# jmoraispk/DeepMIMO

Measured on AMD Instinct MI355X. Metric: user-channels/sec, higher is better.
Workload: dtype f16x3-split MFMA, f32 accumulate

## Files before the change

deepmimo_amd/csrc/k2_channel_fd_fold.hip:

```cpp
#include "dmx_common.h"
#include "dmx_tuning.h"

namespace dmx {

typedef _Float16 fh8 __attribute__((ext_vector_type(8)));
typedef _Float16 fh2 __attribute__((ext_vector_type(2)));
typedef __fp16 fhp2 __attribute__((ext_vector_type(2)));
typedef float ff16 __attribute__((ext_vector_type(16)));
typedef unsigned fu4 __attribute__((ext_vector_type(4)));

static constexpr int FOLD_TROW = 272;
static constexpr float FOLD_B_SCALE = 64.0f;
static constexpr int FOLD_MAX_M = 128;
static constexpr int FOLD_SHARED_FROM = 33;
static constexpr size_t FOLD_MIN_LDS = 160 * 1024 / 5 + 64;

struct FoldArgs {
    int64_t user_begin;
    int m_tx, ue_mh, bs_mh;
    int M, K;
    int sc_first, sc_stride;
    double inv_n;
    int ch;
    int sch;
    int nblk;
    int nchunk;
    int nsuper;
    int nb_last;
    int tab_rows;
    int adaptive;
    int k_tail;
    int mlog;
};

typedef float fv2 __attribute__((ext_vector_type(2)));

__device__ __forceinline__ void fold_split2(float x0, float x1, fh2& hi, fh2& lo, float m1) {
    const fhp2 h = __builtin_amdgcn_cvt_pkrtz(x0, x1);
    const fh2 hh = __builtin_bit_cast(fh2, h);
    const float r0 = __builtin_fmaf((float)hh[0], m1, x0);
    const float r1 = __builtin_fmaf((float)hh[1], m1, x1);
    const fhp2 l = __builtin_amdgcn_cvt_pkrtz(r0, r1);
    hi = hh;
    lo = __builtin_bit_cast(fh2, l);
}

__device__ __forceinline__ unsigned fold_bits(float x) { return __builtin_bit_cast(unsigned, x); }

__device__ __forceinline__ float fold_max_paths(float v) {
    int x = __builtin_bit_cast(int, v);
    v = fmaxf(v, __builtin_bit_cast(float, __builtin_amdgcn_update_dpp(x, x, 0xB1, 0xF, 0xF, false)));
    x = __builtin_bit_cast(int, v);
    v = fmaxf(v, __builtin_bit_cast(float, __builtin_amdgcn_update_dpp(x, x, 0x4E, 0xF, 0xF, false)));
    x = __builtin_bit_cast(int, v);
    v = fmaxf(v, __builtin_bit_cast(float, __builtin_amdgcn_update_dpp(x, x, 0x141, 0xF, 0xF, false)));
    x = __builtin_bit_cast(int, v);
    v = fmaxf(v, __builtin_bit_cast(float, __builtin_amdgcn_update_dpp(x, x, 0x140, 0xF, 0xF, false)));
    x = __builtin_bit_cast(int, v);
    return fmaxf(__builtin_bit_cast(float, __builtin_amdgcn_readlane(x, 0)), __builtin_bit_cast(float, __builtin_amdgcn_readlane(x, 16)));
}

__device__ __forceinline__ void wave_lds_sync() {
    __builtin_amdgcn_fence(__ATOMIC_ACQ_REL, "workgroup");
    __builtin_amdgcn_wave_barrier();
}

__host__ __device__ inline size_t fold_static_bytes(int tab_rows, int M) { return (size_t)tab_rows * 12 + align_up((size_t)M * 4, 16); }
__host__ __device__ inline size_t fold_wave_bytes(int M, int ch) { return 256 + (size_t)(M + ch) * FOLD_TROW; }

template <int WS>
__device__ __forceinline__ void fold_sync() {
    if constexpr (WS == 4) __syncthreads();
    else wave_lds_sync();
}


typedef float ff4 __attribute__((ext_vector_type(4)));
struct FoldX { ff4 x0, x1, y0, y1; };
#define FOLD_X_IO(X) "+{v[112:115]}"((X).x0), "+{v[116:119]}"((X).x1), "+{v[120:123]}"((X).y0), "+{v[124:127]}"((X).y1)

__device__ __forceinline__ uint32_t fold_lds_addr(const void* p) {
    return (uint32_t)(size_t)(__attribute__((address_space(3))) const void*)p;
}

__device__ __forceinline__ void fold_load0(FoldX& X, uint32_t ar, uint32_t er) {
    asm volatile(
        "ds_read_b128 v[112:115], %4\n\t"
        "ds_read_b128 v[116:119], %4 offset:16\n\t"
        "ds_read_b128 v[120:123], %5\n\t"
        "ds_read_b128 v[124:127], %5 offset:16"
        : "={v[112:115]}"(X.x0), "={v[116:119]}"(X.x1), "={v[120:123]}"(X.y0), "={v[124:127]}"(X.y1)
        : "v"(ar), "v"(er));
}

__device__ __forceinline__ void fold_drain(FoldX& X) { asm volatile("s_waitcnt lgkmcnt(0)" : FOLD_X_IO(X)); }

#define FOLD_CMUL_TEXT                                                                                               \
    "s_waitcnt lgkmcnt(0)\n\t"                                                                                       \
    "v_pk_mul_f32 v[108:109], v[112:113], v[120:121] op_sel:[1,1] op_sel_hi:[1,0]\n\t"                                \
    "v_pk_mul_f32 v[110:111], v[114:115], v[122:123] op_sel:[1,1] op_sel_hi:[1,0]\n\t"                                \
    "v_pk_fma_f32 v[112:113], v[112:113], v[120:121], v[108:109] op_sel_hi:[0,1,1] neg_lo:[0,0,1]\n\t"                \
    "v_pk_fma_f32 v[114:115], v[114:115], v[122:123], v[110:111] op_sel_hi:[0,1,1] neg_lo:[0,0,1]\n\t"                \
    "v_pk_mul_f32 v[108:109], v[116:117], v[124:125] op_sel:[1,1] op_sel_hi:[1,0]\n\t"                                \
    "v_pk_mul_f32 v[110:111], v[118:119], v[126:127] op_sel:[1,1] op_sel_hi:[1,0]\n\t"                                \
    "v_pk_fma_f32 v[116:117], v[116:117], v[124:125], v[108:109] op_sel_hi:[0,1,1] neg_lo:[0,0,1]\n\t"                \
    "v_pk_fma_f32 v[118:119], v[118:119], v[126:127], v[110:111] op_sel_hi:[0,1,1] neg_lo:[0,0,1]\n\t"
#define FOLD_CVT_HI_TEXT                                                                                             \
    "v_cvt_pkrtz_f16_f32 %0, v112, v113\n\t"                                                                         \
    "v_cvt_pkrtz_f16_f32 %1, v114, v115\n\t"                                                                         \
    "v_cvt_pkrtz_f16_f32 %2, v116, v117\n\t"                                                                         \
    "v_cvt_pkrtz_f16_f32 %3, v118, v119\n\t"
template <bool LO, int OFF>
__device__ __forceinline__ void fold_kstep(FoldX& X, float m1, uint32_t ar, uint32_t er, fh8& Ah, fh8& Al) {
    unsigned h0, h1, h2, h3;
    if constexpr (LO) {
        unsigned l0, l1, l2, l3;
        asm volatile(
            FOLD_CMUL_TEXT
            FOLD_CVT_HI_TEXT
            "v_fma_mix_f32 v112, %0, %14, v112 op_sel_hi:[1,0,0]\n\t"
            "v_fma_mix_f32 v113, %0, %14, v113 op_sel:[1,0,0] op_sel_hi:[1,0,0]\n\t"
            "v_fma_mix_f32 v114, %1, %14, v114 op_sel_hi:[1,0,0]\n\t"
            "v_fma_mix_f32 v115, %1, %14, v115 op_sel:[1,0,0] op_sel_hi:[1,0,0]\n\t"
            "v_fma_mix_f32 v116, %2, %14, v116 op_sel_hi:[1,0,0]\n\t"
            "v_fma_mix_f32 v117, %2, %14, v117 op_sel:[1,0,0] op_sel_hi:[1,0,0]\n\t"
            "v_fma_mix_f32 v118, %3, %14, v118 op_sel_hi:[1,0,0]\n\t"
            "v_fma_mix_f32 v119, %3, %14, v119 op_sel:[1,0,0] op_sel_hi:[1,0,0]\n\t"
            "v_cvt_pkrtz_f16_f32 %4, v112, v113\n\t"
            "v_cvt_pkrtz_f16_f32 %5, v114, v115\n\t"
            "v_cvt_pkrtz_f16_f32 %6, v116, v117\n\t"
            "v_cvt_pkrtz_f16_f32 %7, v118, v119\n\t"
            "ds_read_b128 v[112:115], %12 offset:%15\n\t"
            "ds_read_b128 v[116:119], %12 offset:%16\n\t"
            "ds_read_b128 v[120:123], %13 offset:%15\n\t"
            "ds_read_b128 v[124:127], %13 offset:%16"
            : "=&v"(h0), "=&v"(h1), "=&v"(h2), "=&v"(h3), "=&v"(l0), "=&v"(l1), "=&v"(l2), "=&v"(l3), FOLD_X_IO(X)
            : "v"(ar), "v"(er), "s"(m1), "i"(OFF), "i"(OFF + 16)
            : "v108", "v109", "v110", "v111");
        Al = __builtin_bit_cast(fh8, fu4{l0, l1, l2, l3});
    } else {
        asm volatile(
            FOLD_CMUL_TEXT
            FOLD_CVT_HI_TEXT
            "ds_read_b128 v[112:115], %8 offset:%10\n\t"
            "ds_read_b128 v[116:119], %8 offset:%11\n\t"
            "ds_read_b128 v[120:123], %9 offset:%10\n\t"
            "ds_read_b128 v[124:127], %9 offset:%11"
            : "=&v"(h0), "=&v"(h1), "=&v"(h2), "=&v"(h3), FOLD_X_IO(X)
            : "v"(ar), "v"(er), "i"(OFF), "i"(OFF + 16)
            : "v108", "v109", "v110", "v111");
    }
    Ah = __builtin_bit_cast(fh8, fu4{h0, h1, h2, h3});
    if constexpr (!LO) Al = Ah;
}
#undef FOLD_CMUL_TEXT
#undef FOLD_CVT_HI_TEXT

__device__ __forceinline__ uint32_t fold_rowbits_off(uint32_t r, int mlog, uint32_t K8) {
    return (r & ((1u << mlog) - 1u)) * K8 + ((r >> mlog) << 7);
}

template <int NS>
__device__ __forceinline__ void fold_finish(ff16& acc0, ff16& acc1, fv2 osc, fv2 (&w)[8]) {
    if constexpr (NS > 1) {
        asm volatile("s_nop 15" : "+v"(acc0), "+v"(acc1));
        fv2 t[8];
#pragma unroll
        for (int i = 0; i < 8; ++i) {
            const fv2 a = {acc0[2 * i], acc0[2 * i + 1]}, b = {acc1[2 * i], acc1[2 * i + 1]};
            asm volatile("v_pk_add_f32 %0, %1, %2" : "=v"(t[i]) : "v"(a), "v"(b));
        }
#pragma unroll
        for (int i = 0; i < 8; ++i) asm volatile("v_pk_mul_f32 %0, %1, %2" : "=v"(w[i]) : "v"(t[i]), "v"(osc));
    } else {
        asm volatile("s_nop 15" : "+v"(acc0));
#pragma unroll
        for (int i = 0; i < 8; ++i) {
            const fv2 a = {acc0[2 * i], acc0[2 * i + 1]};
            asm volatile("v_pk_mul_f32 %0, %1, %2" : "=v"(w[i]) : "v"(a), "v"(osc));
        }
    }
}

template <int S, int NS, bool LW>
__device__ __forceinline__ void fold_ksteps(FoldX& X, float m1, uint32_t ar, uint32_t er, uint32_t arn, uint32_t ern,
                                            ff16& acc0, ff16& acc1, const fh8 (&Bhi)[4], const fh8 (&Blo)[4]) {
    constexpr bool weak = LW && S == NS - 1;
    fh8 Ah, Al;
    if constexpr (S == NS - 1) fold_kstep<!weak, 0>(X, m1, arn, ern, Ah, Al);
    else fold_kstep<true, (S + 1) * 64>(X, m1, ar, er, Ah, Al);
    __builtin_amdgcn_sched_barrier(0);
    if constexpr (S & 1) {
        acc1 = __builtin_amdgcn_mfma_f32_32x32x16_f16(Ah, Bhi[S], acc1, 0, 0, 0);
        if constexpr (!weak) {
            acc1 = __builtin_amdgcn_mfma_f32_32x32x16_f16(Ah, Blo[S], acc1, 0, 0, 0);
            acc1 = __builtin_amdgcn_mfma_f32_32x32x16_f16(Al, Bhi[S], acc1, 0, 0, 0);
        }
    } else {
        acc0 = __builtin_amdgcn_mfma_f32_32x32x16_f16(Ah, Bhi[S], acc0, 0, 0, 0);
        if constexpr (!weak) {
            acc0 = __builtin_amdgcn_mfma_f32_32x32x16_f16(Ah, Blo[S], acc0, 0, 0, 0);
            acc0 = __builtin_amdgcn_mfma_f32_32x32x16_f16(Al, Bhi[S], acc0, 0, 0, 0);
        }
    }
    __builtin_amdgcn_sched_barrier(0);
    if constexpr (S + 1 < NS) fold_ksteps<S + 1, NS, LW>(X, m1, ar, er, arn, ern, acc0, acc1, Bhi, Blo);
}

struct FoldStoreCtx {
    __amdgpu_buffer_rsrc_t orsrc;
    uint32_t lane_col;
    uint32_t lane_row;
    uint32_t lmask_last;
    uint32_t K8;
    int mlog;
    int nb;
    int lane_hh;
    int tail_lane_dead;
    bool masked;
};

template <bool NT, int WS, int NS, bool LW, bool SROW>
__device__ __forceinline__ void fold_tiles(int sub, int ntiles, const uint32_t* rowsrc, const uint32_t* rowoff, int lp, int hh,
                                           const unsigned char* Ac, const unsigned char* E1, const fh8 (&Bhi)[4], const fh8 (&Blo)[4],
                                           float m1, fv2 osc, const FoldStoreCtx& c) {
    if (sub >= ntiles) return;
    constexpr int AUX = NT ? 2 : 0;
    const int rows = c.nb << (SROW ? c.mlog : 0);
    const int rt_chk = !SROW ? 0 : (c.masked ? (((c.nb - 1) << c.mlog) >> 5) : ((rows & 31) ? ntiles - 1 : ntiles));
    uint32_t P[4], D[4];
    if constexpr (SROW) {
#pragma unroll
        for (int q = 0; q < 4; ++q) { P[q] = fold_rowbits_off((uint32_t)q, c.mlog, c.K8); D[q] = fold_rowbits_off((uint32_t)(8 * q), c.mlog, c.K8); }
    }
    const uint32_t ac_lds = fold_lds_addr(Ac) + (uint32_t)hh * 32u, e1_lds = fold_lds_addr(E1) + (uint32_t)hh * 32u;
    uint32_t src = rowsrc[(sub << 5) + lp];
    uint32_t ar = ac_lds + (src >> 16), er = e1_lds + (src & 0xFFFFu);
    FoldX X;
    fold_load0(X, ar, er);
    for (int rt = sub; rt < ntiles; rt += WS) {
        const int rtn = rt + WS < ntiles ? rt + WS : rt;
        const uint32_t srcn = rowsrc[(rtn << 5) + lp];
        const uint32_t arn = ac_lds + (srcn >> 16), ern = e1_lds + (srcn & 0xFFFFu);
        ff16 acc0, acc1;
#pragma unroll
        for (int i = 0; i < 16; ++i) { acc0[i] = 0.f; acc1[i] = 0.f; }
        fold_ksteps<0, NS, LW>(X, m1, ar, er, arn, ern, acc0, acc1, Bhi, Blo);
        ar = arn; er = ern;
        fv2 w[8];
        fold_finish<NS>(acc0, acc1, osc, w);
        if constexpr (SROW) {
            const uint32_t T = fold_rowbits_off((uint32_t)rt << 5, c.mlog, c.K8);
            if (rt < rt_chk) {
#pragma unroll
                for (int i = 0; i < 16; ++i)
                    __builtin_amdgcn_raw_buffer_store_b32(fold_bits(w[i >> 1][i & 1]), c.orsrc, c.lane_row, T + P[i & 3] + D[i >> 2], AUX);
            } else {
#pragma unroll
                for (int i = 0; i < 16; ++i) {
                    const int a_blk = ((rt << 5) + (i & 3) + 8 * (i >> 2) + 4 * c.lane_hh) >> c.mlog;
                    const bool dead = a_blk >= c.nb || (c.masked && a_blk == c.nb - 1 && c.tail_lane_dead);
                    __builtin_amdgcn_raw_buffer_store_b32(fold_bits(w[i >> 1][i & 1]), c.orsrc, dead ? 0x80000000u : c.lane_row,
                                                          T + P[i & 3] + D[i >> 2], AUX);
                }
            }
        } else {
            const uint4* ro4 = reinterpret_cast<const uint4*>(rowoff + (rt << 5) + 4 * hh);
            if (c.masked) {
#pragma unroll
                for (int g = 0; g < 4; ++g) {
                    const uint4 ro = ro4[2 * g];
                    __builtin_amdgcn_raw_buffer_store_b32(fold_bits(w[2 * g][0]), c.orsrc, c.lane_col + (ro.x & c.lmask_last), 0, AUX);
                    __builtin_amdgcn_raw_buffer_store_b32(fold_bits(w[2 * g][1]), c.orsrc, c.lane_col + (ro.y & c.lmask_last), 0, AUX);
                    __builtin_amdgcn_raw_buffer_store_b32(fold_bits(w[2 * g + 1][0]), c.orsrc, c.lane_col + (ro.z & c.lmask_last), 0, AUX);
                    __builtin_amdgcn_raw_buffer_store_b32(fold_bits(w[2 * g + 1][1]), c.orsrc, c.lane_col + (ro.w & c.lmask_last), 0, AUX);
                }
            } else {
#pragma unroll
                for (int g = 0; g < 4; ++g) {
                    const uint4 ro = ro4[2 * g];
                    __builtin_amdgcn_raw_buffer_store_b32(fold_bits(w[2 * g][0]), c.orsrc, c.lane_col + ro.x, 0, AUX);
                    __builtin_amdgcn_raw_buffer_store_b32(fold_bits(w[2 * g][1]), c.orsrc, c.lane_col + ro.y, 0, AUX);
                    __builtin_amdgcn_raw_buffer_store_b32(fold_bits(w[2 * g + 1][0]), c.orsrc, c.lane_col + ro.z, 0, AUX);
                    __builtin_amdgcn_raw_buffer_store_b32(fold_bits(w[2 * g + 1][1]), c.orsrc, c.lane_col + ro.w, 0, AUX);
                }
            }
        }
    }
    fold_drain(X);
}

template <bool NT, int WS, bool SROW>
__device__ __forceinline__ void fold_tiles_kind(int tile_kind, int sub, int ntiles, const uint32_t* rowsrc, const uint32_t* rowoff, int lp, int hh,
                                                const unsigned char* Ac, const unsigned char* E1, const fh8 (&Bhi)[4], const fh8 (&Blo)[4],
                                                float m1, fv2 osc, const FoldStoreCtx& c) {
    switch (tile_kind) {
        case 2: fold_tiles<NT, WS, 1, false, SROW>(sub, ntiles, rowsrc, rowoff, lp, hh, Ac, E1, Bhi, Blo, m1, osc, c); break;
        case 4: fold_tiles<NT, WS, 2, false, SROW>(sub, ntiles, rowsrc, rowoff, lp, hh, Ac, E1, Bhi, Blo, m1, osc, c); break;
        case 5: fold_tiles<NT, WS, 2, true, SROW>(sub, ntiles, rowsrc, rowoff, lp, hh, Ac, E1, Bhi, Blo, m1, osc, c); break;
        case 6: fold_tiles<NT, WS, 3, false, SROW>(sub, ntiles, rowsrc, rowoff, lp, hh, Ac, E1, Bhi, Blo, m1, osc, c); break;
        case 7: fold_tiles<NT, WS, 3, true, SROW>(sub, ntiles, rowsrc, rowoff, lp, hh, Ac, E1, Bhi, Blo, m1, osc, c); break;
        case 8: fold_tiles<NT, WS, 4, false, SROW>(sub, ntiles, rowsrc, rowoff, lp, hh, Ac, E1, Bhi, Blo, m1, osc, c); break;
        default: fold_tiles<NT, WS, 4, true, SROW>(sub, ntiles, rowsrc, rowoff, lp, hh, Ac, E1, Bhi, Blo, m1, osc, c); break;
    }
}

template <bool NT, int WS>
__global__ __launch_bounds__(256, 4) void k2_fd_fold(WsView ws, FoldArgs a, float* __restrict__ out, int64_t items) {
    extern __shared__ __attribute__((aligned(16))) unsigned char smem[];
    uint32_t* rowoff0 = reinterpret_cast<uint32_t*>(smem);
    uint32_t* rowoff1 = rowoff0 + a.tab_rows;
    uint32_t* rowsrc = rowoff1 + a.tab_rows;
    uint32_t* pidx = rowsrc + a.tab_rows;
    const int tid = threadIdx.x, lane = tid & 63;
    const int wave = __builtin_amdgcn_readfirstlane(tid >> 6);
    unsigned char* wbase = smem + fold_static_bytes(a.tab_rows, a.M) + (WS == 1 ? (size_t)wave * fold_wave_bytes(a.M, a.ch) : (size_t)0);
    float2* qtab = reinterpret_cast<float2*>(wbase);
    unsigned char* Ac = wbase + 256;
    unsigned char* E1 = Ac + (size_t)a.M * FOLD_TROW;

    const int M = a.M, K = a.K;
    for (int r = tid; r < a.tab_rows; r += 256) {
        const int ab = r / M, p = r - ab * M;
        const uint32_t off = (uint32_t)(p * K + 16 * ab) * 8u;
        const int nb0 = a.nchunk > 1 ? a.ch : a.nb_last;
        rowoff0[r] = ab < nb0 ? off : 0xC0000000u;
        uint32_t o1 = ab < a.nb_last ? off : 0xC0000000u;
        if (ab == a.nb_last - 1 && a.k_tail < 16) o1 |= 0x80000000u;
        rowoff1[r] = o1;
        const bool any = ab < (a.ch > a.nb_last ? a.ch : a.nb_last);
        rowsrc[r] = any ? ((uint32_t)(ab * FOLD_TROW) | ((uint32_t)(p * FOLD_TROW) << 16)) : 0u;
    }
    for (int p = tid; p < M; p += 256) {
        const int rx = p / a.m_tx, tx = p - rx * a.m_tx;
        pidx[p] = (uint32_t)(rx % a.ue_mh) | ((uint32_t)(rx / a.ue_mh) << 8) | ((uint32_t)(tx % a.bs_mh) << 16) |
                  ((uint32_t)(tx / a.bs_mh) << 24);
    }
    __syncthreads();

    const int lp = lane & 31, hh = lane >> 5;
    const int col = lane & 31, bsc = col >> 1, cpart = col & 1;
    const int kb = a.sc_stride * bsc;
    const float kbl = (float)(kb & 4095), kbf = (float)kb, cq = 0.25f * (float)cpart;
    const uint32_t lane_col = (uint32_t)col * 4u;
    const uint32_t lmask_last = bsc < a.k_tail ? 0x7FFFFFFFu : 0xFFFFFFFFu;
    const size_t user_floats = (size_t)M * K * 2;

    constexpr int IW = 4 / WS;
    const int sub = WS == 4 ? wave : 0;
    for (int64_t item = (int64_t)blockIdx.x * IW + (WS == 1 ? wave : 0); item < items; item += (int64_t)gridDim.x * IW) {
        const int64_t ul = a.nsuper == 1 ? item : item / a.nsuper;
        const int sc = a.nsuper == 1 ? 0 : (int)(item - ul * a.nsuper);
        const int64_t u = a.user_begin + ul;
        const int b0 = sc * a.sch;
        const int bn = (a.nblk - b0) < a.sch ? (a.nblk - b0) : a.sch;
        int n_act = ws.n_keep[u];
        n_act = n_act < 32 ? n_act : 32;
        if (n_act == 0) {
            float* __restrict__ oz = out + (size_t)ul * user_floats + (size_t)b0 * 32;
            const int k0 = b0 * 16, k1 = (k0 + bn * 16) < K ? (k0 + bn * 16) : K;
            const int nfl = (k1 - k0) * 2;
            for (int p = sub; p < M; p += WS)
                for (int i = lane; i < nfl; i += 64) oz[(size_t)p * K * 2 + i] = 0.f;
            continue;
        }
        const size_t rb = (size_t)u * ws.P + lp;
        const bool ok = lp < n_act;
        const float cr = ok ? ws.c_re[rb] : 0.f, ci = ok ? ws.c_im[rb] : 0.f;
        const double q = ok ? (double)ws.dn[rb] * a.inv_n : 0.0;
        const double rxy = ok ? ws.rx_y[rb] : 0.0, rxz = ok ? ws.rx_z[rb] : 0.0;
        const double txy = ok ? ws.tx_y[rb] : 0.0, txz = ok ? ws.tx_z[rb] : 0.0;
        const float m = fold_max_paths(fmaxf(fabsf(cr), fabsf(ci)));
        bool last_weak = false;
        if (a.adaptive) {
            const int l0w = ((n_act - 1) >> 3) << 3;
            const float a2 = fmaf(cr, cr, ci * ci);
            const float m2 = fold_max_paths(a2), mw2 = fold_max_paths(lp >= l0w ? a2 : 0.f);
            last_weak = l0w >= 8 && mw2 * 4194304.0f <= m2;
        }
        int e;
        (void)frexpf(m, &e);
        const float gs = ldexpf(1.0f, 10 - e);
        const float oscale = ldexpf(1.0f, e - 10 - 6);
        const fv2 osc = {oscale, oscale};
        const double qh = rint(q * 4096.0) * (1.0 / 4096.0);
        const float qhf = (float)qh, qlf = (float)(q - qh);
        const float cgr = cr * gs, cgi = ci * gs;
        fold_sync<WS>();
        if (lane < 32 && sub == 0) qtab[lane] = make_float2(qhf, qlf);
        for (int p = 2 * sub + hh; p < M; p += 2 * WS) {
            const uint32_t ix = pidx[p];
            const double ph = (double)(ix & 255u) * rxy + (double)((ix >> 8) & 255u) * rxz +
                              (double)((ix >> 16) & 255u) * txy + (double)(ix >> 24) * txz;
            float s, c;
            sincos_rev(frac_rev(ph), s, c);
            *reinterpret_cast<float2*>(Ac + (size_t)p * FOLD_TROW + lp * 8) = make_float2(cgr * c - cgi * s, cgr * s + cgi * c);
        }
        fold_sync<WS>();

        const int nsteps = (n_act + 7) >> 3;
        const int tile_kind = __builtin_amdgcn_readfirstlane(2 * nsteps + (last_weak ? 1 : 0));
        fh8 Bhi[4], Blo[4];
#pragma unroll
        for (int s = 0; s < 4; ++s) {
            Bhi[s] = fh8{0, 0, 0, 0, 0, 0, 0, 0};
            Blo[s] = Bhi[s];
            if (s < nsteps) {
#pragma unroll
                for (int jj = 0; jj < 4; ++jj) {
                    const float2 qq = qtab[8 * s + 4 * hh + jj];
                    const float p1 = fmaf(qq.x, kbl, cq);
                    float sn, cs;
                    sincos_rev(fmaf(qq.y, kbf, p1 - rintf(p1)), sn, cs);
                    fh2 ph, pl;
                    fold_split2(cs * FOLD_B_SCALE, sn * FOLD_B_SCALE, ph, pl, ws.neg_one);
                    Bhi[s][2 * jj] = ph[0]; Bhi[s][2 * jj + 1] = ph[1];
                    Blo[s][2 * jj] = pl[0]; Blo[s][2 * jj + 1] = pl[1];
                }
            }
        }

        for (int c0 = 0; c0 < bn; c0 += a.ch) {
        const int a0 = b0 + c0;
        const int nb = (bn - c0) < a.ch ? (bn - c0) : a.ch;
        const bool last = a0 + nb == a.nblk;
        float* __restrict__ o = out + (size_t)ul * user_floats + (size_t)a0 * 32;
        fold_sync<WS>();
        {
            const int dsc = a.sc_stride * 32 * WS;
            const float pw = qhf * (float)(dsc & 4095);
            float ws_, wc_;
            sincos_rev(fmaf(qlf, (float)dsc, pw - rintf(pw)), ws_, wc_);
            const float wr = wc_, wi = -ws_;
            float er_ = 1.f, ei_ = 0.f;
            int it = 0;
            for (int ab = 2 * sub + hh; ab < nb; ab += 2 * WS, ++it) {
                if ((it & 7) == 0) {
                    const int sca = a.sc_first + a.sc_stride * 16 * (a0 + ab);
                    const float p1 = qhf * (float)(sca & 4095);
                    float s, c;
                    sincos_rev(fmaf(qlf, (float)sca, p1 - rintf(p1)), s, c);
                    er_ = c; ei_ = -s;
                } else {
                    const float t = fmaf(-ei_, wi, er_ * wr);
                    ei_ = fmaf(ei_, wr, er_ * wi);
                    er_ = t;
                }
                *reinterpret_cast<float2*>(E1 + (size_t)ab * FOLD_TROW + lp * 8) = make_float2(er_, ei_);
            }
        }
        fold_sync<WS>();

        const uint32_t* rowoff = last ? rowoff1 : rowoff0;
        const int rows = nb * M;
        const int ntiles = (rows + 31) >> 5;
        FoldStoreCtx sc_;
        sc_.orsrc = __builtin_amdgcn_make_buffer_rsrc(o, 0, (int)((unsigned)(user_floats - (size_t)a0 * 32) * 4u), 0x00020000);
        sc_.lane_col = lane_col;
        sc_.K8 = (uint32_t)K * 8u;
        sc_.mlog = a.mlog;
        sc_.lane_row = lane_col + (a.mlog >= 0 ? (uint32_t)hh * fold_rowbits_off(4u, a.mlog, (uint32_t)K * 8u) : 0u);
        sc_.lmask_last = lmask_last;
        sc_.nb = nb;
        sc_.lane_hh = hh;
        sc_.tail_lane_dead = bsc >= a.k_tail;
        sc_.masked = last && a.k_tail < 16;
        if (a.mlog >= 0) fold_tiles_kind<NT, WS, true>(tile_kind, sub, ntiles, rowsrc, rowoff, lp, hh, Ac, E1, Bhi, Blo, ws.neg_one, osc, sc_);
        else fold_tiles_kind<NT, WS, false>(tile_kind, sub, ntiles, rowsrc, rowoff, lp, hh, Ac, E1, Bhi, Blo, ws.neg_one, osc, sc_);
        }
    }
}

bool fd_fold_supported(const dmx_params& prm, const WsView& ws) {
    (void)ws;
    const int64_t M = (int64_t)prm.ue_shape[0] * prm.ue_shape[1] * prm.bs_shape[0] * prm.bs_shape[1];
    return prm.sc_stride > 0 && prm.n_selected >= 1 && M <= FOLD_MAX_M;
}

static constexpr int FOLD_SUPER = 64;
static int fold_chunk_blocks(int M, int nblk, int forced, int table_sets) {
    const int cand[3] = {32, 16, 8};
    if (forced > 0) return forced < nblk ? forced : nblk;
    for (int want = 4; want >= 2; --want) {
        for (int ch : cand) {
            const int c = ch < nblk ? ch : nblk;
            const int tab = (M * c + 31) / 32 * 32;
            const size_t smem = fold_static_bytes(tab, M) + table_sets * fold_wave_bytes(M, c);
            if (smem * want <= 160 * 1024) return c;
        }
    }
    return 8 < nblk ? 8 : nblk;
}

bool fd_fold_preferred(const dmx_params& prm, const WsView& ws) {
    const int64_t M = (int64_t)prm.ue_shape[0] * prm.ue_shape[1] * prm.bs_shape[0] * prm.bs_shape[1];
    const int K = prm.n_selected;
    if (!fd_fold_supported(prm, ws) || K < (M <= 16 ? 4 : 6)) return false;
    if (M <= 32) return true;
    if (M <= 48) return K <= 512;
    if (M <= 64) return K <= 256;
    if (M <= 96) return K <= 128;
    return K <= 64;
}

int launch_channels_fd_fold(const dmx_params& prm, const WsView& ws, int64_t user_begin, int64_t user_count, float2* out,
                            int chunk_blocks, hipStream_t stream) {
    if (user_count == 0 || prm.n_selected == 0) return DMX_OK;
    if (!fd_fold_supported(prm, ws)) {
        set_error("the folded kernel needs a uniformly spaced subcarrier selection (dmx_params.sc_stride > 0) and at most %d antenna pairs", FOLD_MAX_M);
        return DMX_ERR_SHAPE;
    }
    FoldArgs a;
    a.user_begin = user_begin;
    a.m_tx = prm.bs_shape[0] * prm.bs_shape[1];
    a.ue_mh = prm.ue_shape[0];
    a.bs_mh = prm.bs_shape[0];
    a.M = prm.ue_shape[0] * prm.ue_shape[1] * a.m_tx;
    a.K = prm.n_selected;
    a.sc_first = prm.sc_first;
    a.sc_stride = prm.sc_stride;
    a.inv_n = 1.0 / (double)prm.n_subcarriers;
    a.nblk = (a.K + 15) / 16;
    if (chunk_blocks <= 0) {
        chunk_blocks = tuning_int("DMX_FOLD_CHUNK", 0);
        if (chunk_blocks != 8 && chunk_blocks != 16 && chunk_blocks != 32) chunk_blocks = 0;
    }
    bool shared = a.M >= FOLD_SHARED_FROM;
    if (const int f = tuning_int("DMX_FOLD_SHARED", -1); f >= 0) shared = f == 1;
    const int sets = shared ? 1 : 4;
    a.ch = fold_chunk_blocks(a.M, a.nblk, chunk_blocks, sets);
    a.sch = (FOLD_SUPER / a.ch) * a.ch;
    if (a.sch > a.nblk) a.sch = (a.nblk + a.ch - 1) / a.ch * a.ch;
    a.nsuper = (a.nblk + a.sch - 1) / a.sch;
    a.nchunk = (a.nblk + a.ch - 1) / a.ch;
    a.nb_last = a.nblk - a.ch * (a.nchunk - 1);
    a.tab_rows = (a.M * a.ch + 31) / 32 * 32;
    a.k_tail = a.K - 16 * (a.nblk - 1);
    a.adaptive = (prm.flags & DMX_FLAG_ADAPTIVE_TERMS) ? 1 : 0;
    a.mlog = -1;
    for (int b = 0; b < 8; ++b) if (a.M == (1 << b)) a.mlog = b;
    if (tuning_int("DMX_FOLD_ROWTABLE", 0) == 1) a.mlog = -1;
    if ((size_t)a.M * (size_t)a.K * 8 >= (size_t)1 << 30) { set_error("%d x %d outputs per user are too many for the folded kernel", a.M, a.K); return DMX_ERR_SHAPE; }
    size_t smem = fold_static_bytes(a.tab_rows, a.M) + sets * fold_wave_bytes(a.M, a.ch);
    if (smem > 160 * 1024) { set_error("folded kernel tables of %zu bytes exceed LDS", smem); return DMX_ERR_SHAPE; }
    if (smem < FOLD_MIN_LDS) smem = FOLD_MIN_LDS;
    const int64_t items = user_count * a.nsuper;
    const void* kfn = shared ? reinterpret_cast<const void*>(k2_fd_fold<true, 4>) : reinterpret_cast<const void*>(k2_fd_fold<true, 1>);
    if (smem > 64 * 1024) {
        hipError_t e = hipFuncSetAttribute(kfn, hipFuncAttributeMaxDynamicSharedMemorySize, (int)smem);
        if (e != hipSuccess) { set_error("hipFuncSetAttribute failed: %s", hipGetErrorString(e)); return DMX_ERR_LAUNCH; }
    }
    int per_cu = 0;
    if (hipOccupancyMaxActiveBlocksPerMultiprocessor(&per_cu, kfn, 256, smem) != hipSuccess || per_cu < 1) {
        (void)hipGetLastError();
        per_cu = 1;
    }
    int64_t grid = (int64_t)device_cu_count() * per_cu;
    const int64_t need = shared ? items : (items + 3) / 4;
    if (grid > need) grid = need;
    if (shared) hipLaunchKernelGGL((k2_fd_fold<true, 4>), dim3((unsigned)grid), dim3(256), smem, stream, ws, a, reinterpret_cast<float*>(out), items);
    else hipLaunchKernelGGL((k2_fd_fold<true, 1>), dim3((unsigned)grid), dim3(256), smem, stream, ws, a, reinterpret_cast<float*>(out), items);
    hipError_t e = hipGetLastError();
    if (e != hipSuccess) { set_error("k2_fd_fold launch failed: %s", hipGetErrorString(e)); return DMX_ERR_LAUNCH; }
    return DMX_OK;
}

}
```

Baseline: 6.387 million.

## Pack hi/lo split of sparse last k-step into a single MFMA

When the final 8-path k-step holds only 1 or 2 active paths, the hi and lo f16 parts of A and B are packed into unused K slots of one MFMA, replacing the three-MFMA split-f16 product with one. The path data is duplicated into the spare lanes so the lo-term products land in the same accumulation, and the adaptive weak-last heuristic is skipped for these cases. This removes two MFMAs per tile for that step, at the cost of more template instantiations (larger code) and slightly different rounding of the packed step.

```diff
diff --git a/deepmimo_amd/csrc/k2_channel_fd_fold.hip b/deepmimo_amd/csrc/k2_channel_fd_fold.hip
--- a/deepmimo_amd/csrc/k2_channel_fd_fold.hip
+++ b/deepmimo_amd/csrc/k2_channel_fd_fold.hip
@@ -156,6 +156,35 @@
 #undef FOLD_CMUL_TEXT
 #undef FOLD_CVT_HI_TEXT
 
+__device__ __forceinline__ void fold_kstep_packed(FoldX& X, float m1, uint32_t ar, uint32_t er, fh8& Ap) {
+    unsigned h0, h1, l0, l1;
+    asm volatile(
+        "s_waitcnt lgkmcnt(0)\n\t"
+        "v_pk_mul_f32 v[108:109], v[112:113], v[120:121] op_sel:[1,1] op_sel_hi:[1,0]\n\t"
+        "v_pk_mul_f32 v[110:111], v[114:115], v[122:123] op_sel:[1,1] op_sel_hi:[1,0]\n\t"
+        "v_pk_fma_f32 v[112:113], v[112:113], v[120:121], v[108:109] op_sel_hi:[0,1,1] neg_lo:[0,0,1]\n\t"
+        "v_pk_fma_f32 v[114:115], v[114:115], v[122:123], v[110:111] op_sel_hi:[0,1,1] neg_lo:[0,0,1]\n\t"
+        "s_nop 3\n\t"
+        "v_cvt_pkrtz_f16_f32 %0, v112, v113\n\t"
+        "v_cvt_pkrtz_f16_f32 %1, v114, v115\n\t"
+        "v_fma_mix_f32 v112, %0, %10, v112 op_sel_hi:[1,0,0]\n\t"
+        "v_fma_mix_f32 v114, %1, %10, v114 op_sel_hi:[1,0,0]\n\t"
+        "v_fma_mix_f32 v113, %0, %10, v113 op_sel:[1,0,0] op_sel_hi:[1,0,0]\n\t"
+        "v_fma_mix_f32 v115, %1, %10, v115 op_sel:[1,0,0] op_sel_hi:[1,0,0]\n\t"
+        "v_cvt_pkrtz_f16_f32 %2, v112, v113\n\t"
+        "v_cvt_pkrtz_f16_f32 %3, v114, v115\n\t"
+        "ds_read_b128 v[112:115], %8\n\t"
+        "ds_read_b128 v[116:119], %8 offset:16\n\t"
+        "ds_read_b128 v[120:123], %9\n\t"
+        "ds_read_b128 v[124:127], %9 offset:16"
+        : "=&v"(h0), "=&v"(h1), "=&v"(l0), "=&v"(l1), FOLD_X_IO(X)
+        : "v"(ar), "v"(er), "s"(m1)
+        : "v108", "v109", "v110", "v111");
+    Ap = __builtin_bit_cast(fh8, fu4{h0, h1, l0, l1});
+}
+
+enum FoldLast { FOLD_LAST_FULL = 0, FOLD_LAST_WEAK = 1, FOLD_LAST_PACKED = 2 };
+
 __device__ __forceinline__ uint32_t fold_rowbits_off(uint32_t r, int mlog, uint32_t K8) {
     return (r & ((1u << mlog) - 1u)) * K8 + ((r >> mlog) << 7);
 }
@@ -182,29 +211,31 @@
     }
 }
 
-template <int S, int NS, bool LW>
+template <int S, int NS, int LM>
 __device__ __forceinline__ void fold_ksteps(FoldX& X, float m1, uint32_t ar, uint32_t er, uint32_t arn, uint32_t ern,
                                             ff16& acc0, ff16& acc1, const fh8 (&Bhi)[4], const fh8 (&Blo)[4]) {
-    constexpr bool weak = LW && S == NS - 1;
+    constexpr bool weak = LM == FOLD_LAST_WEAK && S == NS - 1;
+    constexpr bool packed = LM == FOLD_LAST_PACKED && S == NS - 1;
     fh8 Ah, Al;
-    if constexpr (S == NS - 1) fold_kstep<!weak, 0>(X, m1, arn, ern, Ah, Al);
+    if constexpr (packed) fold_kstep_packed(X, m1, arn, ern, Ah);
+    else if constexpr (S == NS - 1) fold_kstep<!weak, 0>(X, m1, arn, ern, Ah, Al);
     else fold_kstep<true, (S + 1) * 64>(X, m1, ar, er, Ah, Al);
     __builtin_amdgcn_sched_barrier(0);
     if constexpr (S & 1) {
         acc1 = __builtin_amdgcn_mfma_f32_32x32x16_f16(Ah, Bhi[S], acc1, 0, 0, 0);
-        if constexpr (!weak) {
+        if constexpr (!weak && !packed) {
             acc1 = __builtin_amdgcn_mfma_f32_32x32x16_f16(Ah, Blo[S], acc1, 0, 0, 0);
             acc1 = __builtin_amdgcn_mfma_f32_32x32x16_f16(Al, Bhi[S], acc1, 0, 0, 0);
         }
     } else {
         acc0 = __builtin_amdgcn_mfma_f32_32x32x16_f16(Ah, Bhi[S], acc0, 0, 0, 0);
-        if constexpr (!weak) {
+        if constexpr (!weak && !packed) {
             acc0 = __builtin_amdgcn_mfma_f32_32x32x16_f16(Ah, Blo[S], acc0, 0, 0, 0);
             acc0 = __builtin_amdgcn_mfma_f32_32x32x16_f16(Al, Bhi[S], acc0, 0, 0, 0);
         }
     }
     __builtin_amdgcn_sched_barrier(0);
-    if constexpr (S + 1 < NS) fold_ksteps<S + 1, NS, LW>(X, m1, ar, er, arn, ern, acc0, acc1, Bhi, Blo);
+    if constexpr (S + 1 < NS) fold_ksteps<S + 1, NS, LM>(X, m1, ar, er, arn, ern, acc0, acc1, Bhi, Blo);
 }
 
 struct FoldStoreCtx {
@@ -220,7 +251,7 @@
     bool masked;
 };
 
-template <bool NT, int WS, int NS, bool LW, bool SROW>
+template <bool NT, int WS, int NS, int LM, bool SROW>
 __device__ __forceinline__ void fold_tiles(int sub, int ntiles, const uint32_t* rowsrc, const uint32_t* rowoff, int lp, int hh,
                                            const unsigned char* Ac, const unsigned char* E1, const fh8 (&Bhi)[4], const fh8 (&Blo)[4],
                                            float m1, fv2 osc, const FoldStoreCtx& c) {
@@ -245,7 +276,7 @@
         ff16 acc0, acc1;
 #pragma unroll
         for (int i = 0; i < 16; ++i) { acc0[i] = 0.f; acc1[i] = 0.f; }
-        fold_ksteps<0, NS, LW>(X, m1, ar, er, arn, ern, acc0, acc1, Bhi, Blo);
+        fold_ksteps<0, NS, LM>(X, m1, ar, er, arn, ern, acc0, acc1, Bhi, Blo);
         ar = arn; er = ern;
         fv2 w[8];
         fold_finish<NS>(acc0, acc1, osc, w);
@@ -294,15 +325,22 @@
 __device__ __forceinline__ void fold_tiles_kind(int tile_kind, int sub, int ntiles, const uint32_t* rowsrc, const uint32_t* rowoff, int lp, int hh,
                                                 const unsigned char* Ac, const unsigned char* E1, const fh8 (&Bhi)[4], const fh8 (&Blo)[4],
                                                 float m1, fv2 osc, const FoldStoreCtx& c) {
+#define FOLD_TILES_CASE(NS, LM) \
+    case 4 * NS + LM: fold_tiles<NT, WS, NS, LM, SROW>(sub, ntiles, rowsrc, rowoff, lp, hh, Ac, E1, Bhi, Blo, m1, osc, c); break;
     switch (tile_kind) {
-        case 2: fold_tiles<NT, WS, 1, false, SROW>(sub, ntiles, rowsrc, rowoff, lp, hh, Ac, E1, Bhi, Blo, m1, osc, c); break;
-        case 4: fold_tiles<NT, WS, 2, false, SROW>(sub, ntiles, rowsrc, rowoff, lp, hh, Ac, E1, Bhi, Blo, m1, osc, c); break;
-        case 5: fold_tiles<NT, WS, 2, true, SROW>(sub, ntiles, rowsrc, rowoff, lp, hh, Ac, E1, Bhi, Blo, m1, osc, c); break;
-        case 6: fold_tiles<NT, WS, 3, false, SROW>(sub, ntiles, rowsrc, rowoff, lp, hh, Ac, E1, Bhi, Blo, m1, osc, c); break;
-        case 7: fold_tiles<NT, WS, 3, true, SROW>(sub, ntiles, rowsrc, rowoff, lp, hh, Ac, E1, Bhi, Blo, m1, osc, c); break;
-        case 8: fold_tiles<NT, WS, 4, false, SROW>(sub, ntiles, rowsrc, rowoff, lp, hh, Ac, E1, Bhi, Blo, m1, osc, c); break;
-        default: fold_tiles<NT, WS, 4, true, SROW>(sub, ntiles, rowsrc, rowoff, lp, hh, Ac, E1, Bhi, Blo, m1, osc, c); break;
-    }
+        FOLD_TILES_CASE(1, FOLD_LAST_FULL)
+        FOLD_TILES_CASE(1, FOLD_LAST_PACKED)
+        FOLD_TILES_CASE(2, FOLD_LAST_FULL)
+        FOLD_TILES_CASE(2, FOLD_LAST_WEAK)
+        FOLD_TILES_CASE(2, FOLD_LAST_PACKED)
+        FOLD_TILES_CASE(3, FOLD_LAST_FULL)
+        FOLD_TILES_CASE(3, FOLD_LAST_WEAK)
+        FOLD_TILES_CASE(3, FOLD_LAST_PACKED)
+        FOLD_TILES_CASE(4, FOLD_LAST_FULL)
+        FOLD_TILES_CASE(4, FOLD_LAST_PACKED)
+        default: fold_tiles<NT, WS, 4, FOLD_LAST_WEAK, SROW>(sub, ntiles, rowsrc, rowoff, lp, hh, Ac, E1, Bhi, Blo, m1, osc, c); break;
+    }
+#undef FOLD_TILES_CASE
 }
 
 template <bool NT, int WS>
@@ -364,15 +402,19 @@
                 for (int i = lane; i < nfl; i += 64) oz[(size_t)p * K * 2 + i] = 0.f;
             continue;
         }
-        const size_t rb = (size_t)u * ws.P + lp;
-        const bool ok = lp < n_act;
+        const int n_last = n_act & 7;
+        const bool packed = n_last == 1 || n_last == 2;
+        const int l0p = n_act & ~7;
+        const bool dup = packed && (unsigned)(lp - l0p - 4) < (unsigned)n_last;
+        const size_t rb = (size_t)u * ws.P + lp - (dup ? 4 : 0);
+        const bool ok = lp < n_act || dup;
         const float cr = ok ? ws.c_re[rb] : 0.f, ci = ok ? ws.c_im[rb] : 0.f;
         const double q = ok ? (double)ws.dn[rb] * a.inv_n : 0.0;
         const double rxy = ok ? ws.rx_y[rb] : 0.0, rxz = ok ? ws.rx_z[rb] : 0.0;
         const double txy = ok ? ws.tx_y[rb] : 0.0, txz = ok ? ws.tx_z[rb] : 0.0;
         const float m = fold_max_paths(fmaxf(fabsf(cr), fabsf(ci)));
         bool last_weak = false;
-        if (a.adaptive) {
+        if (a.adaptive && !packed) {
             const int l0w = ((n_act - 1) >> 3) << 3;
             const float a2 = fmaf(cr, cr, ci * ci);
             const float m2 = fold_max_paths(a2), mw2 = fold_max_paths(lp >= l0w ? a2 : 0.f);
@@ -399,13 +441,27 @@
         fold_sync<WS>();
 
         const int nsteps = (n_act + 7) >> 3;
-        const int tile_kind = __builtin_amdgcn_readfirstlane(2 * nsteps + (last_weak ? 1 : 0));
+        const int tile_kind = __builtin_amdgcn_readfirstlane(4 * nsteps + (packed ? FOLD_LAST_PACKED : last_weak ? FOLD_LAST_WEAK : FOLD_LAST_FULL));
         fh8 Bhi[4], Blo[4];
 #pragma unroll
         for (int s = 0; s < 4; ++s) {
             Bhi[s] = fh8{0, 0, 0, 0, 0, 0, 0, 0};
             Blo[s] = Bhi[s];
-            if (s < nsteps) {
+            if (packed && s == nsteps - 1) {
+#pragma unroll
+                for (int jj = 0; jj < 2; ++jj) {
+                    const float2 qq = qtab[8 * s + jj];
+                    const float p1 = fmaf(qq.x, kbl, cq);
+                    float sn, cs;
+                    sincos_rev(fmaf(qq.y, kbf, p1 - rintf(p1)), sn, cs);
+                    fh2 ph, pl;
+                    fold_split2(cs * FOLD_B_SCALE, sn * FOLD_B_SCALE, ph, pl, ws.neg_one);
+                    const fh2 z = {0, 0};
+                    const fh2 f = hh ? pl : ph, g = hh ? z : ph;
+                    Bhi[s][2 * jj] = f[0]; Bhi[s][2 * jj + 1] = f[1];
+                    Bhi[s][4 + 2 * jj] = g[0]; Bhi[s][5 + 2 * jj] = g[1];
+                }
+            } else if (s < nsteps) {
 #pragma unroll
                 for (int jj = 0; jj < 4; ++jj) {
                     const float2 qq = qtab[8 * s + 4 * hh + jj];
```

Measured after the change: 6.401 million (median of 5 runs). About the same (+0.2%).
